# WWWindrunner/Cross-Modal-Video-Engine

Measured on AMD Instinct MI355X. Metric: query-video pairs/sec scored + R@1/5/10 parity, MSR-VTT-1kA at 1/8 GPU, higher is better.
Workload: dtype f16

## Files before the change

### cross-modal-video-engine_amd/csrc/cmve_internal.h

```cpp
#pragma once
#include <hip/hip_runtime.h>
#include <hip/hip_ext.h>
#include <stdint.h>
#include <math.h>
#include <string>
#include <algorithm>
#include <type_traits>
#include "../../include/cmve.h"

struct cmve_handle {
  int device;
  hipStream_t stream;
  hipStream_t aux = nullptr;
  hipEvent_t ev[CMVE_MAX_CHUNKS + 2] = {};
  hipEvent_t tev[2 * CMVE_MAX_CHUNKS] = {};
  int last_chunks = 0;
  hipEvent_t eval_ev[CMVE_EVAL_TIMING_SLOTS][4] = {};
  hipEvent_t eval_kev[CMVE_EVAL_TIMING_SLOTS][8] = {};
  bool eval_no_fix[CMVE_EVAL_TIMING_SLOTS] = {};
  bool eval_chained[CMVE_EVAL_TIMING_SLOTS] = {};
  void* scratch = nullptr;
  size_t scratch_bytes = 0;
  void* comm = nullptr;
  int nranks = 1, rank = 0;
// ... 233 lines not shown
  }
  for (int64_t k = lane; k < d; k += WAVE) {
    const double v = (double)x[k];
    ss = fma(v, v, ss);
  }
  return wave_sum(ss);
}
__device__ __forceinline__ double row_inv_norm(double ss, double eps, int flags) {
  const double nrm = sqrt(ss);
  return (flags & CMVE_PACK_RAW) ? 1.0 : (eps > 0.0 ? 1.0 / fmax(nrm, eps) : 1.0 / nrm);
}

struct PackAcc {
  double e1 = 0.0, e2 = 0.0, e3 = 0.0;
  float e4 = 0.f;
};

__device__ __forceinline__ int xcd_linear(int bid, int total) {
  const int xcd = bid & 7, local = bid >> 3;
  const int q = total >> 3, r = total & 7;
  return (xcd < r ? xcd * (q + 1) : r * (q + 1) + (xcd - r) * q) + local;
}

__device__ __forceinline__ uint16_t lo16_elem(float xf, _Float16 h, float& res) {
  const float d2 = xf - (float)h;
  const uint16_t lo = f2bf(d2);
  res = d2 - bf2f(lo);
  return lo;
}
__device__ __forceinline__ float lo16_bound(double ss_res) {
  return f32_round_up(sqrt(ss_res) * (1.0 + 1e-4) + 5.9605e-8 * (1.0 + 1e-6) + 1e-12);
}
__device__ __forceinline__ _Float16 f16_via_f32(double xh, float& xf) {
  xf = (float)xh;
  asm volatile("" : "+v"(xf));
  return (_Float16)xf;
}

__device__ __forceinline__ void pack_elem(double xh, bool want_f16, uint16_t& h, uint16_t& l, uint16_t& f,
                                          PackAcc& acc) {
  float xf;
  const _Float16 hf16 = f16_via_f32(xh, xf);
  if (want_f16) {
    const double r3 = xh - (double)hf16;
    acc.e3 = fma(r3, r3, acc.e3);
    f = __builtin_bit_cast(uint16_t, hf16);
  }
  h = f2bf(xf);
  const float hf = bf2f(h);
  l = f2bf(xf - hf);
  const double r1 = xh - (double)hf;
  const double r2 = r1 - (double)bf2f(l);
  acc.e1 = fma(r1, r1, acc.e1);
// ... 60 lines not shown
}

constexpr int CAND_BUCKET_SHIFT = 8;
struct CandLayout {
  int64_t nb, cap_b;
};
inline CandLayout cand_layout(int64_t g_n_pad, int64_t cap) {
  CandLayout l;
  l.nb = std::max<int64_t>(1, (g_n_pad + (1 << CAND_BUCKET_SHIFT) - 1) >> CAND_BUCKET_SHIFT);
  l.cap_b = cap > l.nb ? (cap - l.nb) / l.nb : 0;
  return l;
}
constexpr int64_t FIXUP_MAX_BUCKETS_PER_XCD = 4096;
constexpr int EVAL_EMAX_SHARDS = 64;

template <typename TA, typename TB, bool LIGHT = false>
__device__ __forceinline__ double wave_cos64(const TA* xa, const TB* xb, double inva, double invb, int64_t d,
                                             int lane) {
  return wave_dot64<TA, TB, LIGHT>(xa, xb, d, lane) * (inva * invb);
}

typedef uint32_t cmve_u32x4 __attribute__((ext_vector_type(4)));
struct L16Frag {
  cmve_u32x4 h0, h1, l0, l1;
};
__device__ __forceinline__ void l16_load(const uint16_t* __restrict__ hrow, const uint16_t* __restrict__ lrow,
                                         int64_t k, L16Frag& f) {
  f.h0 = gld((const cmve_u32x4*)(hrow + k));
  f.h1 = gld((const cmve_u32x4*)(hrow + k + 8));
  f.l0 = gld((const cmve_u32x4*)(lrow + k));
  f.l1 = gld((const cmve_u32x4*)(lrow + k + 8));
}
__device__ __forceinline__ double l16_x(uint32_t hw, uint32_t lw, int half) {
  const uint16_t h = (uint16_t)(hw >> (16 * half));
  const uint32_t l = half ? (lw & 0xffff0000u) : (lw << 16);
  return (double)((float)__builtin_bit_cast(_Float16, h) + __uint_as_float(l));
}
__device__ __forceinline__ double l16_partial(const L16Frag& a, const L16Frag& b) {
  const uint32_t ah[8] = {a.h0.x, a.h0.y, a.h0.z, a.h0.w, a.h1.x, a.h1.y, a.h1.z, a.h1.w};
  const uint32_t al[8] = {a.l0.x, a.l0.y, a.l0.z, a.l0.w, a.l1.x, a.l1.y, a.l1.z, a.l1.w};
  const uint32_t bh[8] = {b.h0.x, b.h0.y, b.h0.z, b.h0.w, b.h1.x, b.h1.y, b.h1.z, b.h1.w};
  const uint32_t bl[8] = {b.l0.x, b.l0.y, b.l0.z, b.l0.w, b.l1.x, b.l1.y, b.l1.z, b.l1.w};
  double acc0 = 0.0, acc1 = 0.0;
#pragma unroll
  for (int w = 0; w < 8; ++w) {
    acc0 = fma(l16_x(ah[w], al[w], 0), l16_x(bh[w], bl[w], 0), acc0);
    acc1 = fma(l16_x(ah[w], al[w], 1), l16_x(bh[w], bl[w], 1), acc1);
  }
  return acc0 + acc1;
}
template <int CTRL>
__device__ __forceinline__ double l16_dpp(double v) {
  const uint64_t b = __builtin_bit_cast(uint64_t, v);
  const uint32_t lo = (uint32_t)__builtin_amdgcn_update_dpp(0, (int)(uint32_t)b, CTRL, 0xF, 0xF, false);
  const uint32_t hi = (uint32_t)__builtin_amdgcn_update_dpp(0, (int)(uint32_t)(b >> 32), CTRL, 0xF, 0xF, false);
  return __builtin_bit_cast(double, (uint64_t)lo | ((uint64_t)hi << 32));
}
__device__ __forceinline__ double l16_wave_sum(double v) {
  v += l16_dpp<0xB1>(v);
  v += l16_dpp<0x4E>(v);
  v += l16_dpp<0x141>(v);
  v += l16_dpp<0x140>(v);
  {
    const uint64_t b = __builtin_bit_cast(uint64_t, v);
    const uint32_t lo = (uint32_t)b, hi = (uint32_t)(b >> 32);
    const auto sl = __builtin_amdgcn_permlane16_swap(lo, lo, false, false);
    const auto sh = __builtin_amdgcn_permlane16_swap(hi, hi, false, false);
    v = __builtin_bit_cast(double, (uint64_t)sl[0] | ((uint64_t)sh[0] << 32)) +
        __builtin_bit_cast(double, (uint64_t)sl[1] | ((uint64_t)sh[1] << 32));
  }
// ... 134 lines not shown
```

### cross-modal-video-engine_amd/csrc/eval.hip

```cpp
#include "eval_abi.h"

namespace cmve {

template <typename T>
__device__ __forceinline__ void load_row_regs(const T* __restrict__ x, int64_t d, int lane, double (&v)[4][4]) {
#pragma unroll
  for (int m = 0; m < 4; ++m) {
    const int64_t k = (int64_t)lane * 4 + 256 * m;
    if (k < d) load4d(x + k, v[m]);
    else v[m][0] = v[m][1] = v[m][2] = v[m][3] = 0.0;
  }
}

__device__ __forceinline__ double lane_sumsq(const double (&v)[4][4], int64_t d, int lane) {
  double ss = 0.0;
#pragma unroll
  for (int m = 0; m < 4; ++m)
    if ((int64_t)lane * 4 + 256 * m < d)
#pragma unroll
      for (int q = 0; q < 4; ++q) ss = fma(v[m][q], v[m][q], ss);
  return ss;
}
__device__ __forceinline__ double lane_dot(const double (&v)[4][4], const double (&w)[4][4], int64_t d, int lane) {
  double dot = 0.0;
// ... 2 lines not shown
    if ((int64_t)lane * 4 + 256 * m < d)
#pragma unroll
      for (int q = 0; q < 4; ++q) dot = fma(v[m][q], w[m][q], dot);
  return dot;
}

template <int K>
__device__ __forceinline__ void wave_sum_k(double (&v)[K]) {
#pragma unroll
  for (int o = 32; o >= 1; o >>= 1)
#pragma unroll
    for (int k = 0; k < K; ++k) v[k] += __shfl_xor(v[k], o, 64);
}

__device__ __forceinline__ void pack_regs_lane(const EvalSide& A, const EvalCommon& c, int64_t row,
                                               const double (&v)[4][4], double inv, int lane, PackAcc& acc);
__device__ __forceinline__ bool pack_bf(const EvalSide& A, const EvalCommon& c) {
  return !(c.mode == CMVE_SIM_F16 && A.h16 != nullptr);
}
__device__ __forceinline__ void pack_bounds(const EvalSide& A, int64_t row, double inv, bool bf, double e1, double e2,
                                            double e3, int lane, float (&eb)[3], double e4 = 0.0) {
  if (lane == 0) {
    gst(A.inv + row, inv);
    if (A.lo16) A.err_lo16[row] = lo16_bound(e4);
    eb[0] = bf ? f32_round_up(sqrt(e1) * (1.0 + 1e-9) + 1e-12) : INFINITY;
    eb[1] = bf ? f32_round_up(sqrt(e2) * (1.0 + 1e-9) + 1e-12) : INFINITY;
    eb[2] = A.err_h16 ? f32_round_up(sqrt(e3) * (1.0 + 1e-9) + 1e-12) : 0.f;
    gst(A.err_hi + row, eb[0]);
    gst(A.err_hilo + row, eb[1]);
    if (A.err_h16) gst(A.err_h16 + row, eb[2]);
  }
}

__device__ __forceinline__ void pack_regs(const EvalSide& A, const EvalCommon& c, int64_t row,
                                          const double (&v)[4][4], double inv, int lane, float (&eb)[3]) {
  PackAcc acc;
  pack_regs_lane(A, c, row, v, inv, lane, acc);
  const bool bf = pack_bf(A, c);
  const double e1 = bf ? wave_sum(acc.e1) : 0.0, e2 = bf ? wave_sum(acc.e2) : 0.0, e3 = wave_sum(acc.e3);
  const double e4 = A.lo16 ? wave_sum((double)acc.e4) : 0.0;
  pack_bounds(A, row, inv, bf, e1, e2, e3, lane, eb, e4);
}

__device__ __forceinline__ void pack_regs_lane(const EvalSide& A, const EvalCommon& c, int64_t row,
                                               const double (&v)[4][4], double inv, int lane, PackAcc& acc) {
  uint16_t* hrow = A.hi + row * c.d_pad;
  uint16_t* lrow = A.lo ? A.lo + row * c.d_pad : nullptr;
  uint16_t* frow = A.h16 ? A.h16 + row * c.d_pad : nullptr;
  const bool want_f16 = frow != nullptr;
  if (c.mode == CMVE_SIM_F16 && want_f16) {
    uint16_t* lrow16 = A.lo16 ? A.lo16 + row * c.d_pad : nullptr;
#pragma unroll
    for (int m = 0; m < 4; ++m) {
      const int64_t k = (int64_t)lane * 4 + 256 * m;
      if (k >= c.d_pad) break;
      cmve_u16x4 fv = {0, 0, 0, 0}, lv = {0, 0, 0, 0};
      if (k < c.d) {
#pragma unroll
        for (int q = 0; q < 4; ++q) {
          const double xh = v[m][q] * inv;
          float xf;
          const _Float16 hf16 = f16_via_f32(xh, xf);
          const double r3 = xh - (double)hf16;
          acc.e3 = fma(r3, r3, acc.e3);
          fv[q] = __builtin_bit_cast(uint16_t, hf16);
          if (lrow16) {
            float res;
            lv[q] = lo16_elem(xf, hf16, res);
            acc.e4 = fmaf(res, res, acc.e4);
          }
        }
      }
      gst((cmve_u16x4*)(frow + k), fv);
      if (lrow16) gst((cmve_u16x4*)(lrow16 + k), lv);
      asm volatile("" : "+v"(acc.e3), "+v"(acc.e4));
    }
  } else {
#pragma unroll
    for (int m = 0; m < 4; ++m) {
      const int64_t k = (int64_t)lane * 4 + 256 * m;
      if (k >= c.d_pad) break;
      cmve_u16x4 hv = {0, 0, 0, 0}, lv = {0, 0, 0, 0}, fv = {0, 0, 0, 0};
      if (k < c.d) {
#pragma unroll
        for (int q = 0; q < 4; ++q) {
          uint16_t h, l, f = 0;
          pack_elem(v[m][q] * inv, want_f16, h, l, f, acc);
          hv[q] = h;
          lv[q] = l;
          fv[q] = f;
        }
      }
      gst((cmve_u16x4*)(hrow + k), hv);
      if (lrow) gst((cmve_u16x4*)(lrow + k), lv);
      if (frow) gst((cmve_u16x4*)(frow + k), fv);
    }
  }
// ... 235 lines not shown
      }
    }
  }
  __shared__ float s_eb[PREP_NW][6];
  if (lane == 0)
#pragma unroll
    for (int k = 0; k < 3; ++k) {
      s_eb[threadIdx.x >> 6][k] = ebq[k];
      s_eb[threadIdx.x >> 6][3 + k] = ebg[k];
    }
  __syncthreads();
  if (threadIdx.x < 6) {
    float m = 0.f;
#pragma unroll
    for (int w = 0; w < PREP_NW; ++w) m = fmaxf(m, s_eb[w][threadIdx.x]);
    unsigned* sh = &c.emax[threadIdx.x * EMAX_SHARDS + blockIdx.x % EMAX_SHARDS];
    if (m == INFINITY) gst(sh, __float_as_uint(m));
    else if (m > 0.f) gmax(sh, __float_as_uint(m));
  }
  EVAL_STAMP(c, 0, 1);
}

template <int NM>
__device__ __forceinline__ void pack_f16_lo16(const EvalSide& A, int64_t row, const double (&v)[NM][4], double inv,
                                              int lane, bool store, double& e3, float& e4) {
  uint16_t* frow = A.h16 + row * (int64_t)(NM * 256);
  uint16_t* lrow = A.lo16 + row * (int64_t)(NM * 256);
  const __amdgpu_buffer_rsrc_t rf = __builtin_amdgcn_make_buffer_rsrc((void*)frow, 0, NM * 512, 0x00020000);
  const __amdgpu_buffer_rsrc_t rl = __builtin_amdgcn_make_buffer_rsrc((void*)lrow, 0, NM * 512, 0x00020000);
  const bool odd = lane & 1;
  cmve_u32x2 pf = {0u, 0u}, pl = {0u, 0u};
  auto swap = [](uint32_t x) { return (uint32_t)__builtin_amdgcn_update_dpp(0, (int)x, 0xB1, 0xF, 0xF, false); };
#pragma unroll
  for (int m = 0; m < NM; ++m) {
    cmve_u16x4 fv, lv;
#pragma unroll
    for (int q = 0; q < 4; ++q) {
      const double xh = v[m][q] * inv;
      float xf;
      const _Float16 h = f16_via_f32(xh, xf);
      const float hf = (float)h;
      const double r3 = xh - (double)hf;
      e3 = fma(r3, r3, e3);
      const float d2 = xf - hf;
      const __bf16 lo = (__bf16)d2;
      const float res = d2 - (float)lo;
      e4 = fmaf(res, res, e4);
      fv[q] = __builtin_bit_cast(uint16_t, h);
      lv[q] = __builtin_bit_cast(uint16_t, lo);
    }
    const cmve_u32x2 f2 = __builtin_bit_cast(cmve_u32x2, fv), l2 = __builtin_bit_cast(cmve_u32x2, lv);
    if (store) {
      if ((m & 1) == 0 && m + 1 < NM) {
        pf = f2;
        pl = l2;
      } else if (m & 1) {
        const cmve_u32x2 sf = odd ? pf : f2, sl = odd ? pl : l2;
        const cmve_u32x2 rf2 = {swap(sf.x), swap(sf.y)}, rl2 = {swap(sl.x), swap(sl.y)};
        const cmve_u32x4 df = odd ? cmve_u32x4{rf2.x, rf2.y, f2.x, f2.y} : cmve_u32x4{pf.x, pf.y, rf2.x, rf2.y};
        const cmve_u32x4 dl = odd ? cmve_u32x4{rl2.x, rl2.y, l2.x, l2.y} : cmve_u32x4{pl.x, pl.y, rl2.x, rl2.y};
        const int off = odd ? (m * 256 + 4 * (lane - 1)) * 2 : ((m - 1) * 256 + 4 * lane) * 2;
        __builtin_amdgcn_raw_buffer_store_b128(df, rf, off, 0, 16);
        __builtin_amdgcn_raw_buffer_store_b128(dl, rl, off, 0, 16);
      } else {
        __builtin_amdgcn_raw_buffer_store_b64(f2, rf, (m * 256 + 4 * lane) * 2, 0, 16);
        __builtin_amdgcn_raw_buffer_store_b64(l2, rl, (m * 256 + 4 * lane) * 2, 0, 16);
      }
    }
    asm volatile("" : "+v"(e3), "+v"(e4));
  }
}

typedef uint32_t prep_u32x4 __attribute__((ext_vector_type(4)));
typedef double prep_f64x2 __attribute__((ext_vector_type(2)));
template <int NM>
__device__ __forceinline__ void load_row_buf(const double* row, int lane, double (&v)[NM][4]) {
  const __amdgpu_buffer_rsrc_t r = __builtin_amdgcn_make_buffer_rsrc((void*)row, 0, NM * 256 * 8, 0x00020000);
#pragma unroll
  for (int m = 0; m < NM; ++m) {
    const prep_f64x2 a = __builtin_bit_cast(prep_f64x2, __builtin_amdgcn_raw_buffer_load_b128(r, lane * 32, m * 2048, 0));
    const prep_f64x2 b =
        __builtin_bit_cast(prep_f64x2, __builtin_amdgcn_raw_buffer_load_b128(r, lane * 32 + 16, m * 2048, 0));
    v[m][0] = a.x;
    v[m][1] = a.y;
    v[m][2] = b.x;
    v[m][3] = b.y;
  }
}
template <int NM>
__device__ __forceinline__ void load_row_buf(const float* row, int lane, double (&v)[NM][4]) {
  const __amdgpu_buffer_rsrc_t r = __builtin_amdgcn_make_buffer_rsrc((void*)row, 0, NM * 256 * 4, 0x00020000);
#pragma unroll
// ... 35 lines not shown
        }
      }
    } else {
      const int64_t qb = gld(q.off + i);
      const int64_t p0 = gld(q.off + i + 1) - qb == 1 ? (int64_t)gld(q.idx + qb) : -1;
      const bool valid = p0 >= 0 && p0 < g.n;
      const int64_t p = valid ? p0 : 0;
      double v[NM][4], w[NM][4];
      load_row_buf<NM>((const TQ*)q.raw + i * q.ld, lane, v);
      load_row_buf<NM>((const TG*)g.raw + p * g.ld, lane, w);
      double r3[3] = {0.0, 0.0, 0.0};
#pragma unroll
      for (int m = 0; m < NM; ++m)
#pragma unroll
        for (int q4 = 0; q4 < 4; ++q4) {
          r3[0] = fma(v[m][q4], v[m][q4], r3[0]);
          r3[1] = fma(w[m][q4], w[m][q4], r3[1]);
          r3[2] = fma(v[m][q4], w[m][q4], r3[2]);
        }
      wave_sum_k<3>(r3);
      const double invq = row_inv_norm(r3[0], q.eps, q.flags), invg = row_inv_norm(r3[1], g.eps, g.flags);
      double e3q = 0.0, e3g = 0.0;
      float e4q = 0.f, e4g = 0.f;
      pack_f16_lo16<NM>(q, i, v, invq, lane, true, e3q, e4q);
      __builtin_amdgcn_sched_barrier(0);
      pack_f16_lo16<NM>(g, p, w, invg, lane, valid, e3g, e4g);
      double e[4] = {e3q, e3g, (double)e4q, (double)e4g};
      wave_sum_k<4>(e);
      pack_bounds(q, i, invq, false, 0.0, 0.0, e[0], lane, ebq, e[2]);
      if (valid) pack_bounds(g, p, invg, false, 0.0, 0.0, e[1], lane, ebg, e[3]);
      const double sc = r3[2] * (invq * invg);
      if (lane == 0) {
        gst(q.sgt + i, !valid ? (double)NAN : (sc == sc ? sc : (double)INFINITY));
        gst(q.cnt + i, 0);
        if (q.gt1) gst(q.gt1 + i, valid ? (int32_t)p : -2);
        if (valid) {
          gst(g.sgt + p, sc == sc ? sc : (double)INFINITY);
          gst(g.cnt + p, 0);
          if (g.gt1) gst(g.gt1 + p, (int32_t)i);
        }
      }
    }
  }
  __shared__ float s_eb[PREP_NW][6];
  if (lane == 0)
#pragma unroll
    for (int k = 0; k < 3; ++k) {
      s_eb[threadIdx.x >> 6][k] = ebq[k];
      s_eb[threadIdx.x >> 6][3 + k] = ebg[k];
// ... 186 lines not shown
__global__ __launch_bounds__(FIN_NT) void eval_finish_batch_kernel(const EvalItem* __restrict__ tab) {
  const EvalItem& it = tab[blockIdx.y];
  eval_finish_body<TQ, TG>(it.q, it.g, it.c, blockIdx.x, gridDim.x);
}
template <typename TQ, typename TG, int NM>
#ifndef CMVE_PREPFIN_WPE
#define CMVE_PREPFIN_WPE 4
#endif
__global__ __launch_bounds__(PREP_NT, CMVE_PREPFIN_WPE) void eval_prep_fin_batch_kernel(const EvalItem* __restrict__ ptab,
                                                                                    const EvalItem* __restrict__ ftab,
                                                                                    int nprep, int nfin) {
  static_assert(PREP_NT == FIN_NT, "one block size for both roles");
  const int bx = (int)blockIdx.x;
  if (bx < nprep) {
    const EvalItem& it = ptab[blockIdx.y];
    eval_prep_pair_f16_body<TQ, TG, NM>(it.q, it.g, it.c, blockIdx.x, nprep);
  } else if (bx < nprep + nfin) {
    const EvalItem& it = ftab[blockIdx.y];
    eval_finish_body<TQ, TG, true>(it.q, it.g, it.c, bx - nprep, nfin);
  }
}

static int prep_f16_nm(const EvalSide& q, const EvalSide& g, const EvalCommon& c) {
  const bool ok = c.mode == CMVE_SIM_F16 && q.h16 && g.h16 && q.lo16 && g.lo16 && q.vec && g.vec && c.d == c.d_pad &&
                  c.d_pad % 256 == 0 && c.d_pad <= 1024;
  return ok ? (int)(c.d_pad / 256) : 0;
}
#define CMVE_PREP_F16(KER, NMV, ...)                                                                            \
  switch (NMV) {                                                                                                \
    case 1: cmve::launch(KER<TQ, TG, 1>, __VA_ARGS__); break;                                                  \
    case 2: cmve::launch(KER<TQ, TG, 2>, __VA_ARGS__); break;                                                  \
    case 3: cmve::launch(KER<TQ, TG, 3>, __VA_ARGS__); break;                                                  \
    default: cmve::launch(KER<TQ, TG, 4>, __VA_ARGS__); break;                                                 \
  }

template <typename TQ, typename TG>
static int launch_eval_batch_typed(const EvalSide& q, const EvalSide& g, const EvalCommon& c0, const EvalItem* tab,
                                   int count, int phase, hipStream_t s) {
  if (phase == 0) {
    const unsigned blocks = (unsigned)((q.n_pad + g.n_pad + PREP_NW - 1) / PREP_NW);
    cmve::launch(eval_prep_batch_kernel<TQ, TG>, dim3(blocks, (unsigned)count), dim3(PREP_NT), 0u, s, tab);
    return check_launch("eval_prep_batch_kernel");
  }
  if (phase == 3) {
    const unsigned blocks = (unsigned)((q.n_pad + PREP_NW - 1) / PREP_NW);
    if (const int nm = prep_f16_nm(q, g, c0)) {
      CMVE_PREP_F16(eval_prep_pair_f16_batch_kernel, nm, dim3(blocks, (unsigned)count), dim3(PREP_NT), 0u, s, tab);
// ... 78 lines not shown
```

### cross-modal-video-engine_amd/csrc/eval_abi.h

```cpp
#pragma once
#include "cmve_internal.h"

namespace cmve {

constexpr int EVAL_ARRIVAL_WORDS = 9 * 64;
constexpr int EMAX_SHARDS = EVAL_EMAX_SHARDS;

struct EvalSide {
  const void* raw;
  int64_t ld;
  int64_t n, n_pad;
  int vec;
  int flags;
  double eps;
  uint16_t* hi;
  uint16_t* lo;
  uint16_t* h16;
  double* inv;
  float* err_hi;
  float* err_hilo;
  float* err_h16;
  float* err_max;
  const int64_t* off;
  const int32_t* idx;
  double* sgt;
  float* thr_hi;
  float* thr_lo;
  int32_t* cnt;
  int64_t* ranks;
  int32_t* gt1;
  uint16_t* lo16;
  float* err_lo16;
};

struct EvalCommon {
  int64_t d, d_pad;
  int mode;
  unsigned* emax;
  unsigned long long* bucket;
  int64_t nb, cap_b;
  const uint64_t* cand;
  int64_t* stats;
  int fix_inline;
  unsigned* l3_count;
  uint64_t* l3;
  int l3_cap;
  unsigned long long* stamps;
};

#define EVAL_STAMP(cp, kern, k)                                                                                  \
  if ((cp).stamps && threadIdx.x == 0 && blockIdx.x < 1024)                                                     \
  (cp).stamps[((size_t)(kern) * 1024 + blockIdx.x) * 8 + (k)] = __builtin_amdgcn_s_memrealtime()
int launch_eval(const EvalSide& q, const EvalSide& g, const EvalCommon& c, int q_f64, int g_f64, int phase,
                hipStream_t s);
struct EvalItem {
// ... 11 lines not shown
```

### cross-modal-video-engine_amd/csrc/sim.hip

```cpp
#include <algorithm>
#include <vector>

#include <hip/hip_ext.h>

#include "cmve_internal.h"

#ifndef CMVE_SIM_GN
#define CMVE_SIM_GN 8
#endif
#ifndef CMVE_EVAL_DBG
#define CMVE_EVAL_DBG 0
#endif
namespace cmve {

typedef __bf16 bf16x8_t __attribute__((ext_vector_type(8)));
typedef _Float16 f16x8_t __attribute__((ext_vector_type(8)));
typedef short s16x8_t __attribute__((ext_vector_type(8)));
typedef float f32x4_t __attribute__((ext_vector_type(4)));
typedef __attribute__((address_space(3))) void lds_void_t;

constexpr int BK = 64;
constexpr int EPI_STORE = 0, EPI_RANK = 1, EPI_LINEAR = 2, EPI_TOPK = 3, EPI_BIAS = 4;
constexpr bool epi_thr(int e) { return e == EPI_RANK || e == EPI_TOPK; }

// ... 28 lines not shown
  long long cand_cap;
  unsigned long long* cand_count;
  unsigned long long* bucket_cnt;
  long long cap_b;
  int thr_gt;
  const double* row_sgt;
  const double* col_sgt;
  const float* q_err;
  const float* g_err;
  const unsigned* q_emax;
  const unsigned* g_emax;
  unsigned long long* dbg_stamps;
  int tile_buckets;
  int nbn64;
  const int* row_gt1;
  const int* col_gt1;
  int fix_inline;
  int q_f64, g_f64;
  const void* q_raw;
  const void* g_raw;
  int64_t q_ld, g_ld, d;
  const double* q_inv;
  const double* g_inv;
  const uint16_t* q_lo16;
  const uint16_t* g_lo16;
  const float* q_el;
  const float* g_el;
  unsigned* l3_count;
  unsigned long long* l3;
  int l3_cap;
};

__device__ __forceinline__ void tile_grouped(int L, int nblk_m, int nblk_n, int GN, int& bm, int& bn);
__device__ __forceinline__ void tile_of_block(int bid, int nblk_m, int nblk_n, int GN, int& bm, int& bn) {
  tile_grouped(xcd_linear(bid, nblk_m * nblk_n), nblk_m, nblk_n, GN, bm, bn);
}
__device__ __forceinline__ void tile_grouped(int L, int nblk_m, int nblk_n, int GN, int& bm, int& bn) {
  const int group = L / (GN * nblk_m);
  const int within = L - group * (GN * nblk_m);
  const int gn = min(GN, nblk_n - group * GN);
  bm = within / gn;
  bn = group * GN + (within - bm * gn);
}

__host__ __device__ constexpr int lds_swz(int r) { return r & 7; }

__device__ __forceinline__ uint32_t stage_lane_off(int64_t ldk, int lane) {
  constexpr int CPR = BK / 8;
// ... 625 lines not shown
          for (int w = 0; w < NWT; ++w) {
            const int t = epi.wtot[w];
            woff += w < wave ? t : 0;
            ntot += t;
          }
          bool listed = ntot <= CMVE_INL_LIST;
          if (listed && nmine) {
            uint32_t slot = (uint32_t)woff + excl;
#pragma unroll
            for (int i = 0; i < TM; ++i) {
              uint32_t m = (und[i] | (und[i] >> 16)) & 0xffffu;
              while (m) {
                const int bit = __builtin_ctz(m);
                m &= m - 1u;
                const uint32_t lr = (uint32_t)(rbase - m0 + i * 16 + (bit & 3));
                const uint32_t lc = (uint32_t)(cbase - n0 + (bit >> 2) * 16);
                const uint32_t fl = ((und[i] >> bit) & 1u) | (((und[i] >> (16 + bit)) & 1u) << 1);
                epi.list[slot++] = lr | (lc << 8) | (fl << 16);
              }
            }
          }
          if (listed) {
            CMVE_BAR_LDS();
            if (a.q_lo16) {
              struct L2Stage {
                float elq, elg;
                L16Frag fq, fg;
              };
              static_assert(!INL || ring_lds_bytes<MODE, BM, BN, PHASED>() >= (size_t)CMVE_INL_LIST * 16,
                            "the level-2 scores alias the staging ring");
              const int64_t l2_ldk = a.ldk;
              const bool l2_inrow = 16 * (int64_t)lane < l2_ldk;
              const int64_t l2_k = l2_inrow ? 16 * (int64_t)lane : 0;
              auto l2_fetch = [&](int p, L2Stage& st) {
                const uint32_t ent = epi.list[p];
                const int64_t qr = m0 + (ent & 0xff), gc = n0 + ((ent >> 8) & 0xff);
                st.elq = gld(a.q_el + qr);
                st.elg = gld(a.g_el + gc);
                l16_load(a.qhi + qr * l2_ldk, a.q_lo16 + qr * l2_ldk, l2_k, st.fq);
                l16_load(a.ghi + gc * l2_ldk, a.g_lo16 + gc * l2_ldk, l2_k, st.fg);
                __builtin_amdgcn_sched_barrier(0);
              };
              auto l2_finish = [&](int p, const L2Stage& st) {
                const double part = l16_partial(st.fq, st.fg);
                const double s2 = l16_wave_sum(l2_inrow ? part : 0.0);
                if (lane == 0) {
                  const uint64_t sb = __builtin_bit_cast(uint64_t, s2);
                  const cmve_u32x4 rec = {(uint32_t)sb, (uint32_t)(sb >> 32), __float_as_uint(st.elq),
                                          __float_as_uint(st.elg)};
                  lds_write_b128_async(smem + 16 * p, rec);
                }
              };
              auto l2_decide = [&]() {
                for (int t0 = 0; t0 < ntot; t0 += NTT) {
                  const int t = t0 + tid;
                  uint32_t ent = 0u, fl = 0u;
                  if (t < ntot) {
                    ent = epi.list[t];
                    const cmve_u32x4 rec = *(const cmve_u32x4*)(smem + 16 * t);
                    const double s2 = __builtin_bit_cast(double, (uint64_t)rec.x | ((uint64_t)rec.y << 32));
                    const double eq = (double)__uint_as_float(rec.z), eg = (double)__uint_as_float(rec.w);
                    const double E2 = eq + (1.0 + eq) * eg + 2e-12;
                    fl = (ent >> 16) & 3u;
// ... 85 lines not shown
              }
            };
            if constexpr (BATCH) {
              for (int p = wave; p < ntot; p += NWT) {
                const uint32_t e = epi.list[p];
                if (!(e >> 16)) continue;
                const int64_t r1 = m0 + (e & 0xff), c1 = n0 + ((e >> 8) & 0xff);
                const double inva = gld(a.q_inv + r1), invb = gld(a.g_inv + c1);
                double s1;
                if (a.q_f64) {
                  const double* x = (const double*)a.q_raw + r1 * a.q_ld;
                  s1 = a.g_f64 ? wave_cos64(x, (const double*)a.g_raw + c1 * a.g_ld, inva, invb, a.d, lane)
                               : wave_cos64(x, (const float*)a.g_raw + c1 * a.g_ld, inva, invb, a.d, lane);
                } else {
                  const float* x = (const float*)a.q_raw + r1 * a.q_ld;
                  s1 = a.g_f64 ? wave_cos64(x, (const double*)a.g_raw + c1 * a.g_ld, inva, invb, a.d, lane)
                               : wave_cos64(x, (const float*)a.g_raw + c1 * a.g_ld, inva, invb, a.d, lane);
                }
                if (lane == 0) {
                  if ((e >> 16) & 1u) { if (s1 > epi.sgt[r1 - m0]) lds_add_u32_async(&lds_rc[r1 - m0], 1); }
                  if ((e >> 17) & 1u) { if (s1 > epi.sgt[BM + c1 - n0]) lds_add_u32_async(&lds_cc[c1 - n0], 1); }
                }
              }
            } else if (a.q_lo16) {
              for (int p = wave; p < ntot; p += NWT) {
                const uint32_t e = epi.list[p];
                if (e >> 16) rescore2(e, 0u, false);
              }
            } else {
              for (int p = 2 * wave; p < ntot; p += 2 * NWT)
                rescore2(epi.list[p], p + 1 < ntot ? epi.list[p + 1] : 0u, p + 1 < ntot);
            }
          } else {
#pragma unroll
            for (int i = 0; i < TM; ++i) {
              uint32_t bits = (und[i] | (und[i] >> 16)) & 0xffffu;
              unsigned long long m;
              while ((m = __builtin_amdgcn_ballot_w64(bits != 0u))) {
                const int src = (int)__builtin_ctzll(m);
                const uint32_t sb = (uint32_t)__builtin_amdgcn_readlane((int)bits, src);
                const uint32_t su = (uint32_t)__builtin_amdgcn_readlane((int)und[i], src);
                const int bit = __builtin_ctz(sb);
                if (lane == src) bits &= bits - 1u;
                const int lr = wr * (TM * 16) + (src >> 4) * 4 + i * 16 + (bit & 3);
                const int lc = wc * (TN * 16) + (src & 15) + (bit >> 2) * 16;
                const int64_t row = m0 + lr, col = n0 + lc;
                const double inva = gld(a.q_inv + row), invb = gld(a.g_inv + col);
// ... 727 lines not shown
  if (st) return st;
  CMVE_REQUIRE(out && ldo >= w->n, "cmve_linear: bad output");
  CMVE_REQUIRE((bn_scale == nullptr) == (bn_shift == nullptr), "cmve_linear: bn_scale and bn_shift go together");
  CMVE_REQUIRE(!resid || ldr >= w->n, "cmve_linear: bad residual leading dimension");
  CMVE_REQUIRE(relu >= 0 && relu <= 3, "cmve_linear: unknown activation %d", relu);
  if (x->n == 0 || w->n == 0) return CMVE_OK;
  SimArgs a = make_args(x, w, mode);
  a.out = out;
  a.ldo = ldo;
  a.bias = bias;
  a.bn_scale = bn_scale;
  a.bn_shift = bn_shift;
  a.resid = resid;
  a.ldr = ldr;
  a.relu = relu;
  if (!resid && !bn_scale && relu <= 1) return dispatch<EPI_BIAS>(a, x, w, mode, h->stream);
  return dispatch<EPI_LINEAR>(a, x, w, mode, h->stream);
}

#include "eval_abi.h"

namespace {
struct EvalWs {
  size_t done, q_sgt, q_hi, q_lo, q_cnt, g_sgt, g_hi, g_lo, g_cnt, q_gt1, g_gt1, q_el, g_el, q_l16, g_l16, l3, cand,
      total;
};
constexpr int EVAL_L3_CAP = 4096;
EvalWs eval_ws_layout(int64_t nq_pad, int64_t ng_pad, int64_t d_pad, int64_t cand_cap) {
  auto up = [](size_t x) { return (x + 255) & ~(size_t)255; };
  EvalWs w;
  size_t o = 0;
  w.done = o;
  o = up(o + 2 * sizeof(unsigned) * cmve::EVAL_ARRIVAL_WORDS);
  w.q_sgt = o;
  o = up(o + 8 * (size_t)nq_pad);
  w.q_hi = o;
  o = up(o + 4 * (size_t)nq_pad);
  w.q_lo = o;
  o = up(o + 4 * (size_t)nq_pad);
  w.q_cnt = o;
  o = up(o + 4 * (size_t)nq_pad);
  w.g_sgt = o;
  o = up(o + 8 * (size_t)ng_pad);
  w.g_hi = o;
  o = up(o + 4 * (size_t)ng_pad);
  w.g_lo = o;
  o = up(o + 4 * (size_t)ng_pad);
  w.g_cnt = o;
  o = up(o + 4 * (size_t)ng_pad);
  w.q_gt1 = o;
  o = up(o + 4 * (size_t)nq_pad);
  w.g_gt1 = o;
  o = up(o + 4 * (size_t)ng_pad);
  w.q_el = o;
  o = up(o + 4 * (size_t)nq_pad);
  w.g_el = o;
  o = up(o + 4 * (size_t)ng_pad);
  w.q_l16 = o;
  o = up(o + 2 * (size_t)nq_pad * (size_t)d_pad);
  w.g_l16 = o;
  o = up(o + 2 * (size_t)ng_pad * (size_t)d_pad);
  w.l3 = o;
  o = up(o + 8 + 8 * (size_t)EVAL_L3_CAP);
  w.cand = o;
  o = up(o + 8 * (size_t)cand_cap);
  w.total = o;
  return w;
}
}

static unsigned long long* g_eval_stamps = nullptr;
extern "C" int cmve_eval_debug_stamps(void* host, int64_t bytes) {
  CMVE_REQUIRE(g_eval_stamps && host, "cmve_eval_debug_stamps: no stamps (CMVE_EVAL_DBG & 128)");
  CMVE_HIP(hipDeviceSynchronize());
  CMVE_HIP(hipMemcpy(host, g_eval_stamps, std::min<int64_t>(bytes, sizeof(unsigned long long) * 4 * 1024 * 8),
                     hipMemcpyDeviceToHost));
  return CMVE_OK;
}

extern "C" int cmve_eval_workspace(const cmve_rows_t* q, const cmve_rows_t* g, int64_t cand_cap, int64_t* bytes) {
  CMVE_REQUIRE(q && g && bytes, "cmve_eval_workspace: NULL argument");
  CMVE_REQUIRE(cand_cap > 0, "cmve_eval_workspace: cand_cap must be > 0");
  *bytes = (int64_t)eval_ws_layout(q->n_pad, g->n_pad, q->d_pad, cand_cap).total;
  return CMVE_OK;
// ... 139 lines not shown
    a.row_lo = P.sq.thr_lo;
    a.row_sgt = P.sq.sgt;
    a.row_cnt = P.sq.cnt;
  }
  if (col_off) {
    a.col_hi = P.sg.thr_hi;
    a.col_lo = P.sg.thr_lo;
    a.col_sgt = P.sg.sgt;
    a.col_cnt = P.sg.cnt;
  }
  set_cand(a, g, cand, cand_cap, out + 10);
  a.bucket_cnt = (unsigned long long*)cand;
  a.cand = (unsigned long long*)(cand + l.nb);
  a.cap_b = l.cap_b;
  a.tile_buckets = tile_buckets;
  a.nbn64 = (int)(g->n_pad >> 6);
  if (a.thr_gt) {
    a.row_gt1 = P.sq.gt1;
    a.col_gt1 = P.sg.gt1;
  }
  P.inline_fix = a.thr_gt && sim_uses_g64(q->n_pad, g->n_pad);
  const bool l2 = P.inline_fix && mode == CMVE_SIM_F16 && P.sq.vec && P.sg.vec && q->d_pad <= 1024;
  if (l2) {
    P.sq.lo16 = (uint16_t*)(base + w.q_l16);
    P.sg.lo16 = (uint16_t*)(base + w.g_l16);
    P.sq.err_lo16 = (float*)(base + w.q_el);
    P.sg.err_lo16 = (float*)(base + w.g_el);
    a.q_lo16 = P.sq.lo16;
    a.g_lo16 = P.sg.lo16;
    a.q_el = P.sq.err_lo16;
    a.g_el = P.sg.err_lo16;
    c.l3_count = (unsigned*)(base + w.l3);
    c.l3 = (uint64_t*)(base + w.l3 + 8);
    c.l3_cap = batch ? EVAL_L3_CAP : 0;
    a.l3_count = c.l3_count;
    a.l3 = batch ? (unsigned long long*)c.l3 : nullptr;
    a.l3_cap = c.l3_cap;
  }
  if (P.inline_fix) {
    a.fix_inline = 1;
    a.q_f64 = P.qf;
    a.g_f64 = P.gf;
    a.q_raw = q->raw;
    a.g_raw = g->raw;
    a.q_ld = q->raw_ld;
    a.g_ld = g->raw_ld;
    a.d = q->d;
    a.q_inv = q->inv_norm;
    a.g_inv = g->inv_norm;
    c.fix_inline = 1;
  }
  a.dbg_stamps = c.stamps ? c.stamps + 3 * 1024 * 8 : nullptr;
  return CMVE_OK;
}
// ... 114 lines not shown
  std::vector<cmve::EvalItem> items((size_t)count);
  std::vector<SimArgs> args((size_t)count);
  EvalPlan P0;
  for (int i = 0; i < count; ++i) {
    EvalPlan P;
    const int st = eval_prepare(q[i], g[i], mode_flags, row_off, row_idx, col_off, col_idx, ws[i], ws_bytes,
                                cand_cap, out[i], "cmve_eval_batch_create", P, true);
    if (st) return st;
    CMVE_REQUIRE(P.inline_fix, "cmve_eval_batch_create: batches take the G64 geometry (fewer than 128 tiles of "
                               "128^2, e.g. 1,000 x 1,000) with the inline fix-up");
    if (P.c.stamps) {
      const int64_t per = (q[i]->n_pad / batch_geo_bm(q[i]->n_pad)) *
                          (g[i]->n_pad / batch_geo_bn(q[i]->n_pad, g[i]->n_pad, mode_flags & 0xff));
      P.a.dbg_stamps = (i + 1) * per <= 1024 ? P.c.stamps + 3 * 1024 * 8 + (size_t)i * per * 8 : nullptr;
      if (i > 0) P.c.stamps = nullptr;
    }
    if (i == 0) {
      P0 = P;
    } else {
      CMVE_REQUIRE(q[i]->n == q[0]->n && g[i]->n == g[0]->n && q[i]->n_pad == q[0]->n_pad &&
                       g[i]->n_pad == g[0]->n_pad && q[i]->d == q[0]->d && q[i]->d_pad == q[0]->d_pad &&
                       P.qf == P0.qf && P.gf == P0.gf && P.paired == P0.paired,
                   "cmve_eval_batch_create: evaluation %d differs in shape / dtype / pairing from the first", i);
      CMVE_REQUIRE(P.sq.vec == P0.sq.vec && P.sg.vec == P0.sg.vec && (P.sq.lo16 != nullptr) == (P0.sq.lo16 != nullptr) &&
                       (P.sg.lo16 != nullptr) == (P0.sg.lo16 != nullptr) &&
                       (P.c.l3_count != nullptr) == (P0.c.l3_count != nullptr),
                   "cmve_eval_batch_create: evaluation %d's inputs take another path than the first's (row alignment "
                   "or stride: every evaluation of a batch needs 16-B aligned rows if the first has them)", i);
      for (int j = 0; j < i; ++j)
        CMVE_REQUIRE(ws[j] != ws[i] && out[j] != out[i],
                     "cmve_eval_batch_create: evaluations %d and %d share a workspace or an output", j, i);
    }
    items[(size_t)i] = cmve::EvalItem{P.sq, P.sg, P.c};
    geo_fill(P.a, q[i]->n_pad, g[i]->n_pad, batch_geo_bm(q[i]->n_pad),
             batch_geo_bn(q[i]->n_pad, g[i]->n_pad, mode_flags & 0xff));
    args[(size_t)i] = P.a;
  }
  auto* b = new cmve_eval_batch;
  b->count = count;
  b->qf = P0.qf;
  b->gf = P0.gf;
  b->mode = mode_flags & 0xff;
  b->paired = P0.paired;
  b->nq_pad = q[0]->n_pad;
  b->ng_pad = g[0]->n_pad;
  b->bm = batch_geo_bm(b->nq_pad);
  b->bn = batch_geo_bn(b->nq_pad, b->ng_pad, b->mode);
  b->sq0 = P0.sq;
// ... 202 lines not shown
```

Before: 139.8 billion.

## Replace bf16 low-residual plane with scaled int8 residual for rescoring

Swaps the 16-bit bf16 residual stored alongside the f16 high part for an 8-bit quantized residual whose scale comes from the f16 element's exponent. Packing, the store shuffles and the second-level rescoring loader and decoder are rewritten to match, and the workspace for the residual planes is halved. The aim is to cut memory traffic and footprint in the pack and inline fix-up stages. In exchange the residual is coarser, so the error bound (err_lo8) is looser, which may send more candidates to the exact fallback. Decoding also costs a little more ALU work per element.

```diff
diff --git a/cross-modal-video-engine_amd/csrc/cmve_internal.h b/cross-modal-video-engine_amd/csrc/cmve_internal.h
--- a/cross-modal-video-engine_amd/csrc/cmve_internal.h
+++ b/cross-modal-video-engine_amd/csrc/cmve_internal.h
@@ -279,13 +279,21 @@
   return (xcd < r ? xcd * (q + 1) : r * (q + 1) + (xcd - r) * q) + local;
 }
 
-__device__ __forceinline__ uint16_t lo16_elem(float xf, _Float16 h, float& res) {
-  const float d2 = xf - (float)h;
-  const uint16_t lo = f2bf(d2);
-  res = d2 - bf2f(lo);
-  return lo;
-}
-__device__ __forceinline__ float lo16_bound(double ss_res) {
+__device__ __forceinline__ uint32_t lo8_scale_bits(float hf) {
+  return max(__float_as_uint(hf) & 0x7f800000u, 113u << 23) - (18u << 23);
+}
+__device__ __forceinline__ float lo8_elem(float xf, float hf, float& res) {
+  const uint32_t sb = lo8_scale_bits(hf);
+  const float d2 = xf - hf;
+  const float q = __builtin_amdgcn_fmed3f(__builtin_rintf(d2 * __uint_as_float((254u << 23) - sb)), -128.f, 127.f);
+  res = fmaf(-q, __uint_as_float(sb), d2);
+  return q;
+}
+__device__ __forceinline__ uint32_t lo8_put(uint32_t w, int c, float q) {
+  return __builtin_amdgcn_cvt_pk_u8_f32(q + 128.f, (uint32_t)c, w);
+}
+constexpr uint32_t LO8_ZERO4 = 0x80808080u;
+__device__ __forceinline__ float lo8_bound(double ss_res) {
   return f32_round_up(sqrt(ss_res) * (1.0 + 1e-4) + 5.9605e-8 * (1.0 + 1e-6) + 1e-12);
 }
 __device__ __forceinline__ _Float16 f16_via_f32(double xh, float& xf) {
@@ -392,30 +400,33 @@
 
 typedef uint32_t cmve_u32x4 __attribute__((ext_vector_type(4)));
 struct L16Frag {
-  cmve_u32x4 h0, h1, l0, l1;
+  cmve_u32x4 h0, h1, r;
 };
-__device__ __forceinline__ void l16_load(const uint16_t* __restrict__ hrow, const uint16_t* __restrict__ lrow,
+__device__ __forceinline__ void l16_load(const uint16_t* __restrict__ hrow, const uint8_t* __restrict__ rrow,
                                          int64_t k, L16Frag& f) {
   f.h0 = gld((const cmve_u32x4*)(hrow + k));
   f.h1 = gld((const cmve_u32x4*)(hrow + k + 8));
-  f.l0 = gld((const cmve_u32x4*)(lrow + k));
-  f.l1 = gld((const cmve_u32x4*)(lrow + k + 8));
-}
-__device__ __forceinline__ double l16_x(uint32_t hw, uint32_t lw, int half) {
-  const uint16_t h = (uint16_t)(hw >> (16 * half));
-  const uint32_t l = half ? (lw & 0xffff0000u) : (lw << 16);
-  return (double)((float)__builtin_bit_cast(_Float16, h) + __uint_as_float(l));
+  f.r = gld((const cmve_u32x4*)(rrow + k));
+}
+template <int E>
+__device__ __forceinline__ double l16_x(uint32_t hw, uint32_t rw) {
+  const float hf = (float)__builtin_bit_cast(_Float16, (uint16_t)(hw >> (16 * (E & 1))));
+  const float sc = __uint_as_float(lo8_scale_bits(hf));
+  const float u = (float)((rw >> (8 * (E & 3))) & 0xffu);
+  return (double)fmaf(u, sc, fmaf(-128.f, sc, hf));
 }
 __device__ __forceinline__ double l16_partial(const L16Frag& a, const L16Frag& b) {
   const uint32_t ah[8] = {a.h0.x, a.h0.y, a.h0.z, a.h0.w, a.h1.x, a.h1.y, a.h1.z, a.h1.w};
-  const uint32_t al[8] = {a.l0.x, a.l0.y, a.l0.z, a.l0.w, a.l1.x, a.l1.y, a.l1.z, a.l1.w};
+  const uint32_t ar[4] = {a.r.x, a.r.y, a.r.z, a.r.w};
   const uint32_t bh[8] = {b.h0.x, b.h0.y, b.h0.z, b.h0.w, b.h1.x, b.h1.y, b.h1.z, b.h1.w};
-  const uint32_t bl[8] = {b.l0.x, b.l0.y, b.l0.z, b.l0.w, b.l1.x, b.l1.y, b.l1.z, b.l1.w};
+  const uint32_t br[4] = {b.r.x, b.r.y, b.r.z, b.r.w};
   double acc0 = 0.0, acc1 = 0.0;
 #pragma unroll
-  for (int w = 0; w < 8; ++w) {
-    acc0 = fma(l16_x(ah[w], al[w], 0), l16_x(bh[w], bl[w], 0), acc0);
-    acc1 = fma(l16_x(ah[w], al[w], 1), l16_x(bh[w], bl[w], 1), acc1);
+  for (int w = 0; w < 8; w += 2) {
+    acc0 = fma(l16_x<0>(ah[w], ar[w / 2]), l16_x<0>(bh[w], br[w / 2]), acc0);
+    acc1 = fma(l16_x<1>(ah[w], ar[w / 2]), l16_x<1>(bh[w], br[w / 2]), acc1);
+    acc0 = fma(l16_x<2>(ah[w + 1], ar[w / 2]), l16_x<2>(bh[w + 1], br[w / 2]), acc0);
+    acc1 = fma(l16_x<3>(ah[w + 1], ar[w / 2]), l16_x<3>(bh[w + 1], br[w / 2]), acc1);
   }
   return acc0 + acc1;
 }
diff --git a/cross-modal-video-engine_amd/csrc/eval.hip b/cross-modal-video-engine_amd/csrc/eval.hip
--- a/cross-modal-video-engine_amd/csrc/eval.hip
+++ b/cross-modal-video-engine_amd/csrc/eval.hip
@@ -48,7 +48,7 @@
                                             double e3, int lane, float (&eb)[3], double e4 = 0.0) {
   if (lane == 0) {
     gst(A.inv + row, inv);
-    if (A.lo16) A.err_lo16[row] = lo16_bound(e4);
+    if (A.lo8) A.err_lo8[row] = lo8_bound(e4);
     eb[0] = bf ? f32_round_up(sqrt(e1) * (1.0 + 1e-9) + 1e-12) : INFINITY;
     eb[1] = bf ? f32_round_up(sqrt(e2) * (1.0 + 1e-9) + 1e-12) : INFINITY;
     eb[2] = A.err_h16 ? f32_round_up(sqrt(e3) * (1.0 + 1e-9) + 1e-12) : 0.f;
@@ -64,7 +64,7 @@
   pack_regs_lane(A, c, row, v, inv, lane, acc);
   const bool bf = pack_bf(A, c);
   const double e1 = bf ? wave_sum(acc.e1) : 0.0, e2 = bf ? wave_sum(acc.e2) : 0.0, e3 = wave_sum(acc.e3);
-  const double e4 = A.lo16 ? wave_sum((double)acc.e4) : 0.0;
+  const double e4 = A.lo8 ? wave_sum((double)acc.e4) : 0.0;
   pack_bounds(A, row, inv, bf, e1, e2, e3, lane, eb, e4);
 }
 
@@ -75,13 +75,15 @@
   uint16_t* frow = A.h16 ? A.h16 + row * c.d_pad : nullptr;
   const bool want_f16 = frow != nullptr;
   if (c.mode == CMVE_SIM_F16 && want_f16) {
-    uint16_t* lrow16 = A.lo16 ? A.lo16 + row * c.d_pad : nullptr;
+    uint8_t* lrow8 = A.lo8 ? A.lo8 + row * c.d_pad : nullptr;
 #pragma unroll
     for (int m = 0; m < 4; ++m) {
       const int64_t k = (int64_t)lane * 4 + 256 * m;
       if (k >= c.d_pad) break;
-      cmve_u16x4 fv = {0, 0, 0, 0}, lv = {0, 0, 0, 0};
+      cmve_u16x4 fv = {0, 0, 0, 0};
+      uint32_t lw = LO8_ZERO4;
       if (k < c.d) {
+        lw = 0u;
 #pragma unroll
         for (int q = 0; q < 4; ++q) {
           const double xh = v[m][q] * inv;
@@ -90,15 +92,15 @@
           const double r3 = xh - (double)hf16;
           acc.e3 = fma(r3, r3, acc.e3);
           fv[q] = __builtin_bit_cast(uint16_t, hf16);
-          if (lrow16) {
+          if (lrow8) {
             float res;
-            lv[q] = lo16_elem(xf, hf16, res);
+            lw = lo8_put(lw, q, lo8_elem(xf, (float)hf16, res));
             acc.e4 = fmaf(res, res, acc.e4);
           }
         }
       }
       gst((cmve_u16x4*)(frow + k), fv);
-      if (lrow16) gst((cmve_u16x4*)(lrow16 + k), lv);
+      if (lrow8) gst((uint32_t*)(lrow8 + k), lw);
       asm volatile("" : "+v"(acc.e3), "+v"(acc.e4));
     }
   } else {
@@ -380,18 +382,23 @@
 }
 
 template <int NM>
-__device__ __forceinline__ void pack_f16_lo16(const EvalSide& A, int64_t row, const double (&v)[NM][4], double inv,
-                                              int lane, bool store, double& e3, float& e4) {
-  uint16_t* frow = A.h16 + row * (int64_t)(NM * 256);
-  uint16_t* lrow = A.lo16 + row * (int64_t)(NM * 256);
+__device__ __forceinline__ void pack_f16_lo8(const EvalSide& A, int64_t row, const double (&v)[NM][4], double inv,
+                                             int lane, bool store, double& e3, float& e4) {
+  const int64_t urow = (int64_t)__builtin_amdgcn_readfirstlane((int)row);
+  uint16_t* frow = A.h16 + urow * (int64_t)(NM * 256);
+  uint8_t* lrow = A.lo8 + urow * (int64_t)(NM * 256);
   const __amdgpu_buffer_rsrc_t rf = __builtin_amdgcn_make_buffer_rsrc((void*)frow, 0, NM * 512, 0x00020000);
-  const __amdgpu_buffer_rsrc_t rl = __builtin_amdgcn_make_buffer_rsrc((void*)lrow, 0, NM * 512, 0x00020000);
-  const bool odd = lane & 1;
-  cmve_u32x2 pf = {0u, 0u}, pl = {0u, 0u};
+  const __amdgpu_buffer_rsrc_t rl = __builtin_amdgcn_make_buffer_rsrc((void*)lrow, 0, NM * 256, 0x00020000);
+  const bool odd = lane & 1, up = lane & 2;
+  const int pair_off = odd ? 512 + 8 * (lane - 1) : 8 * lane;
+  cmve_u32x2 pf = {0u, 0u};
+  uint32_t lw[NM];
   auto swap = [](uint32_t x) { return (uint32_t)__builtin_amdgcn_update_dpp(0, (int)x, 0xB1, 0xF, 0xF, false); };
+  auto swap2 = [](uint32_t x) { return (uint32_t)__builtin_amdgcn_update_dpp(0, (int)x, 0x4E, 0xF, 0xF, false); };
 #pragma unroll
   for (int m = 0; m < NM; ++m) {
-    cmve_u16x4 fv, lv;
+    cmve_u16x4 fv;
+    lw[m] = 0u;
 #pragma unroll
     for (int q = 0; q < 4; ++q) {
       const double xh = v[m][q] * inv;
@@ -400,32 +407,40 @@
       const float hf = (float)h;
       const double r3 = xh - (double)hf;
       e3 = fma(r3, r3, e3);
-      const float d2 = xf - hf;
-      const __bf16 lo = (__bf16)d2;
-      const float res = d2 - (float)lo;
+      float res;
+      lw[m] = lo8_put(lw[m], q, lo8_elem(xf, hf, res));
       e4 = fmaf(res, res, e4);
       fv[q] = __builtin_bit_cast(uint16_t, h);
-      lv[q] = __builtin_bit_cast(uint16_t, lo);
-    }
-    const cmve_u32x2 f2 = __builtin_bit_cast(cmve_u32x2, fv), l2 = __builtin_bit_cast(cmve_u32x2, lv);
+    }
+    const cmve_u32x2 f2 = __builtin_bit_cast(cmve_u32x2, fv);
     if (store) {
       if ((m & 1) == 0 && m + 1 < NM) {
         pf = f2;
-        pl = l2;
       } else if (m & 1) {
-        const cmve_u32x2 sf = odd ? pf : f2, sl = odd ? pl : l2;
-        const cmve_u32x2 rf2 = {swap(sf.x), swap(sf.y)}, rl2 = {swap(sl.x), swap(sl.y)};
+        const cmve_u32x2 sf = odd ? pf : f2;
+        const cmve_u32x2 rf2 = {swap(sf.x), swap(sf.y)};
         const cmve_u32x4 df = odd ? cmve_u32x4{rf2.x, rf2.y, f2.x, f2.y} : cmve_u32x4{pf.x, pf.y, rf2.x, rf2.y};
-        const cmve_u32x4 dl = odd ? cmve_u32x4{rl2.x, rl2.y, l2.x, l2.y} : cmve_u32x4{pl.x, pl.y, rl2.x, rl2.y};
-        const int off = odd ? (m * 256 + 4 * (lane - 1)) * 2 : ((m - 1) * 256 + 4 * lane) * 2;
-        __builtin_amdgcn_raw_buffer_store_b128(df, rf, off, 0, 16);
-        __builtin_amdgcn_raw_buffer_store_b128(dl, rl, off, 0, 16);
+        __builtin_amdgcn_raw_buffer_store_b128(df, rf, pair_off + (m - 1) * 512, 0, 16);
       } else {
-        __builtin_amdgcn_raw_buffer_store_b64(f2, rf, (m * 256 + 4 * lane) * 2, 0, 16);
-        __builtin_amdgcn_raw_buffer_store_b64(l2, rl, (m * 256 + 4 * lane) * 2, 0, 16);
-      }
-    }
-    asm volatile("" : "+v"(e3), "+v"(e4));
+        __builtin_amdgcn_raw_buffer_store_b64(f2, rf, 8 * lane + m * 512, 0, 16);
+      }
+      if constexpr (NM == 4) {
+        if (m == 3) {
+          const uint32_t x0 = swap(odd ? lw[0] : lw[1]), x1 = swap(odd ? lw[2] : lw[3]);
+          const uint32_t a0 = odd ? x0 : lw[0], a1 = odd ? lw[1] : x0, a2 = odd ? x1 : lw[2], a3 = odd ? lw[3] : x1;
+          const uint32_t y0 = swap2(up ? a0 : a2), y1 = swap2(up ? a1 : a3);
+          const cmve_u32x4 dl = up ? cmve_u32x4{y0, y1, a2, a3} : cmve_u32x4{a0, a1, y0, y1};
+          __builtin_amdgcn_raw_buffer_store_b128(dl, rl, (lane & 3) * 256 + 16 * (lane >> 2), 0, 16);
+        }
+      } else if (m & 1) {
+        const uint32_t x = swap(odd ? lw[m - 1] : lw[m]);
+        const cmve_u32x2 dl = odd ? cmve_u32x2{x, lw[m]} : cmve_u32x2{lw[m - 1], x};
+        __builtin_amdgcn_raw_buffer_store_b64(dl, rl, (pair_off >> 1) + (m - 1) * 256, 0, 16);
+      } else if (m + 1 == NM) {
+        __builtin_amdgcn_raw_buffer_store_b32(lw[m], rl, 4 * lane + m * 256, 0, 16);
+      }
+    }
+    asm volatile("" : "+v"(e3), "+v"(e4), "+v"(lw[m]));
   }
 }
 
@@ -507,9 +522,9 @@
       const double invq = row_inv_norm(r3[0], q.eps, q.flags), invg = row_inv_norm(r3[1], g.eps, g.flags);
       double e3q = 0.0, e3g = 0.0;
       float e4q = 0.f, e4g = 0.f;
-      pack_f16_lo16<NM>(q, i, v, invq, lane, true, e3q, e4q);
+      pack_f16_lo8<NM>(q, i, v, invq, lane, true, e3q, e4q);
       __builtin_amdgcn_sched_barrier(0);
-      pack_f16_lo16<NM>(g, p, w, invg, lane, valid, e3g, e4g);
+      pack_f16_lo8<NM>(g, p, w, invg, lane, valid, e3g, e4g);
       double e[4] = {e3q, e3g, (double)e4q, (double)e4g};
       wave_sum_k<4>(e);
       pack_bounds(q, i, invq, false, 0.0, 0.0, e[0], lane, ebq, e[2]);
@@ -742,7 +757,7 @@
 }
 
 static int prep_f16_nm(const EvalSide& q, const EvalSide& g, const EvalCommon& c) {
-  const bool ok = c.mode == CMVE_SIM_F16 && q.h16 && g.h16 && q.lo16 && g.lo16 && q.vec && g.vec && c.d == c.d_pad &&
+  const bool ok = c.mode == CMVE_SIM_F16 && q.h16 && g.h16 && q.lo8 && g.lo8 && q.vec && g.vec && c.d == c.d_pad &&
                   c.d_pad % 256 == 0 && c.d_pad <= 1024;
   return ok ? (int)(c.d_pad / 256) : 0;
 }
diff --git a/cross-modal-video-engine_amd/csrc/eval_abi.h b/cross-modal-video-engine_amd/csrc/eval_abi.h
--- a/cross-modal-video-engine_amd/csrc/eval_abi.h
+++ b/cross-modal-video-engine_amd/csrc/eval_abi.h
@@ -29,8 +29,8 @@
   int32_t* cnt;
   int64_t* ranks;
   int32_t* gt1;
-  uint16_t* lo16;
-  float* err_lo16;
+  uint8_t* lo8;
+  float* err_lo8;
 };
 
 struct EvalCommon {
diff --git a/cross-modal-video-engine_amd/csrc/sim.hip b/cross-modal-video-engine_amd/csrc/sim.hip
--- a/cross-modal-video-engine_amd/csrc/sim.hip
+++ b/cross-modal-video-engine_amd/csrc/sim.hip
@@ -74,8 +74,8 @@
   int64_t q_ld, g_ld, d;
   const double* q_inv;
   const double* g_inv;
-  const uint16_t* q_lo16;
-  const uint16_t* g_lo16;
+  const uint8_t* q_lo8;
+  const uint8_t* g_lo8;
   const float* q_el;
   const float* g_el;
   unsigned* l3_count;
@@ -747,7 +747,7 @@
           }
           if (listed) {
             CMVE_BAR_LDS();
-            if (a.q_lo16) {
+            if (a.q_lo8) {
               struct L2Stage {
                 float elq, elg;
                 L16Frag fq, fg;
@@ -762,8 +762,8 @@
                 const int64_t qr = m0 + (ent & 0xff), gc = n0 + ((ent >> 8) & 0xff);
                 st.elq = gld(a.q_el + qr);
                 st.elg = gld(a.g_el + gc);
-                l16_load(a.qhi + qr * l2_ldk, a.q_lo16 + qr * l2_ldk, l2_k, st.fq);
-                l16_load(a.ghi + gc * l2_ldk, a.g_lo16 + gc * l2_ldk, l2_k, st.fg);
+                l16_load(a.qhi + qr * l2_ldk, a.q_lo8 + qr * l2_ldk, l2_k, st.fq);
+                l16_load(a.ghi + gc * l2_ldk, a.g_lo8 + gc * l2_ldk, l2_k, st.fg);
                 __builtin_amdgcn_sched_barrier(0);
               };
               auto l2_finish = [&](int p, const L2Stage& st) {
@@ -895,7 +895,7 @@
                   if ((e >> 17) & 1u) { if (s1 > epi.sgt[BM + c1 - n0]) lds_add_u32_async(&lds_cc[c1 - n0], 1); }
                 }
               }
-            } else if (a.q_lo16) {
+            } else if (a.q_lo8) {
               for (int p = wave; p < ntot; p += NWT) {
                 const uint32_t e = epi.list[p];
                 if (e >> 16) rescore2(e, 0u, false);
@@ -1669,7 +1669,7 @@
 
 namespace {
 struct EvalWs {
-  size_t done, q_sgt, q_hi, q_lo, q_cnt, g_sgt, g_hi, g_lo, g_cnt, q_gt1, g_gt1, q_el, g_el, q_l16, g_l16, l3, cand,
+  size_t done, q_sgt, q_hi, q_lo, q_cnt, g_sgt, g_hi, g_lo, g_cnt, q_gt1, g_gt1, q_el, g_el, q_l8, g_l8, l3, cand,
       total;
 };
 constexpr int EVAL_L3_CAP = 4096;
@@ -1703,10 +1703,10 @@
   o = up(o + 4 * (size_t)nq_pad);
   w.g_el = o;
   o = up(o + 4 * (size_t)ng_pad);
-  w.q_l16 = o;
-  o = up(o + 2 * (size_t)nq_pad * (size_t)d_pad);
-  w.g_l16 = o;
-  o = up(o + 2 * (size_t)ng_pad * (size_t)d_pad);
+  w.q_l8 = o;
+  o = up(o + (size_t)nq_pad * (size_t)d_pad);
+  w.g_l8 = o;
+  o = up(o + (size_t)ng_pad * (size_t)d_pad);
   w.l3 = o;
   o = up(o + 8 + 8 * (size_t)EVAL_L3_CAP);
   w.cand = o;
@@ -1892,14 +1892,14 @@
   P.inline_fix = a.thr_gt && sim_uses_g64(q->n_pad, g->n_pad);
   const bool l2 = P.inline_fix && mode == CMVE_SIM_F16 && P.sq.vec && P.sg.vec && q->d_pad <= 1024;
   if (l2) {
-    P.sq.lo16 = (uint16_t*)(base + w.q_l16);
-    P.sg.lo16 = (uint16_t*)(base + w.g_l16);
-    P.sq.err_lo16 = (float*)(base + w.q_el);
-    P.sg.err_lo16 = (float*)(base + w.g_el);
-    a.q_lo16 = P.sq.lo16;
-    a.g_lo16 = P.sg.lo16;
-    a.q_el = P.sq.err_lo16;
-    a.g_el = P.sg.err_lo16;
+    P.sq.lo8 = (uint8_t*)(base + w.q_l8);
+    P.sg.lo8 = (uint8_t*)(base + w.g_l8);
+    P.sq.err_lo8 = (float*)(base + w.q_el);
+    P.sg.err_lo8 = (float*)(base + w.g_el);
+    a.q_lo8 = P.sq.lo8;
+    a.g_lo8 = P.sg.lo8;
+    a.q_el = P.sq.err_lo8;
+    a.g_el = P.sg.err_lo8;
     c.l3_count = (unsigned*)(base + w.l3);
     c.l3 = (uint64_t*)(base + w.l3 + 8);
     c.l3_cap = batch ? EVAL_L3_CAP : 0;
@@ -2060,8 +2060,8 @@
                        g[i]->n_pad == g[0]->n_pad && q[i]->d == q[0]->d && q[i]->d_pad == q[0]->d_pad &&
                        P.qf == P0.qf && P.gf == P0.gf && P.paired == P0.paired,
                    "cmve_eval_batch_create: evaluation %d differs in shape / dtype / pairing from the first", i);
-      CMVE_REQUIRE(P.sq.vec == P0.sq.vec && P.sg.vec == P0.sg.vec && (P.sq.lo16 != nullptr) == (P0.sq.lo16 != nullptr) &&
-                       (P.sg.lo16 != nullptr) == (P0.sg.lo16 != nullptr) &&
+      CMVE_REQUIRE(P.sq.vec == P0.sq.vec && P.sg.vec == P0.sg.vec && (P.sq.lo8 != nullptr) == (P0.sq.lo8 != nullptr) &&
+                       (P.sg.lo8 != nullptr) == (P0.sg.lo8 != nullptr) &&
                        (P.c.l3_count != nullptr) == (P0.c.l3_count != nullptr),
                    "cmve_eval_batch_create: evaluation %d's inputs take another path than the first's (row alignment "
                    "or stride: every evaluation of a batch needs 16-B aligned rows if the first has them)", i);
```

New measurement: 145.6 billion (median of 6 runs). +4.2%, better.
